# reonaledo/Multi-modality-Self-supervision

Hardware: AMD Instinct MI355X
Metric: image-text pairs/sec pretraining step, BERT-base seq512 (higher is better)
Workload: dtype f16

## Files before the change

include/medvill.h:

```cpp
#ifndef MEDVILL_H_
#define MEDVILL_H_

#include <stddef.h>
#include <stdint.h>

#ifdef __cplusplus
extern "C" {
#endif

#define MV_ABI_VERSION 6

enum { MV_F32 = 0, MV_BF16 = 1, MV_F16 = 2 };

enum {
  MV_OK = 0,
  MV_E_ARG = -1,
  MV_E_SHAPE = -2,
  MV_E_DTYPE = -3,
  MV_E_WORKSPACE = -4,
  MV_E_NO_RCCL = -5,
  MV_E_COMM_BASE = -1000
};

enum {
// ... 102 lines not shown

int mv_ce_fwd_bwd(const void* logits, int l_dtype, int ld, const int32_t* labels, int R, int V,
                  float* out, void* dlogits, int d_dtype, int ldd,
                  const float* grad_scale_dev, float grad_scale_host, const float* loss_scale_dev, void* stream);

int mv_gather_rows(int dtype, const void* src, int lds, const int32_t* rows, int R, int H,
                   void* dst, int ldd, void* stream);
int mv_scatter_rows(int dtype, const void* src, int lds, const int32_t* rows, int R, int H,
                    void* dst, int ldd, int accumulate, void* stream);

int mv_colsum(int dtype, const void* x, int ldx, int M, int N, float* out, int accumulate, const float* grad_unscale_dev,
              void* stream);
int mv_colsum_partials(const float* part, int P, int ld, int N, float* out, const float* grad_unscale_dev, void* stream);

int mv_add(int dtype, const void* a, const void* b, void* c, size_t n, void* stream);

int mv_dact(int dtype, int mode, const void* dy, const void* z, void* out, size_t n, void* stream);

int mv_cast2d(const void* src, int src_dtype, long long lds, void* dst, int dst_dtype, long long ldd,
              int rows, int cols, void* stream);

int mv_transpose(int dtype, const void* src, long long lds, void* dst, long long ldd, int rows, int cols, void* stream);

int mv_cast(const void* src, int src_dtype, void* dst, int dst_dtype, size_t n, void* stream);

int mv_nchw_to_nhwc(const float* src, void* dst, int dst_dtype, int B, int C, int H, int W, int Cp, void* stream);
int mv_im2col(int dtype, const void* src, int B, int H, int W, int C, int kh, int kw, int stride, int pad, void* dst, int ldk,
              void* stream);
int mv_conv2d(int dtype, const void* x, const void* w, void* y, int y_dtype, int B, int H, int W, int C, int O, int kh, int kw,
              int stride, int pad, const float* bias, int epi, const void* R, int r_dtype, void* stream);
int mv_col_stats(int dtype, const void* x, int ldx, int rows, int C, float* stats, void* stream);
int mv_bn_finalize(const float* stats, int C, long long rows, float eps, float momentum, float* mean, float* rstd,
                   float* running_mean, float* running_var, void* stream);
int mv_bn_act(int dtype, const void* x, int x_dtype, const float* mean, const float* rstd, const float* gamma, const float* beta,
              const void* residual, void* y, long long rows, int C, int relu, void* stream);
int mv_maxpool3x3s2(int dtype, const void* x, void* y, int B, int H, int W, int C, void* stream);

int mv_dropout_mask(float p_drop, unsigned long long drop_key, size_t n, uint8_t* keep, float* scale_out,
                    void* stream);

int mv_adamw_step(float* p, const float* g, float* m, float* v, void* shadow_bf16, void* shadow_f16, size_t n,
                  float lr, float beta1, float beta2, float eps, float weight_decay, int step,
                  int correct_bias, float grad_scale, const float* scaler_state, void* stream);

int mv_count_nonfinite(const float* x, size_t n, float* counter, void* stream);
int mv_scaler_update(float* state, int growth_interval, float growth, float backoff, float max_scale, float min_scale,
// ... 54 lines not shown
```

multi-modality-self-supervision_amd/_lib.py:

```python
from __future__ import annotations

import ctypes as C
import os

import torch

HERE = os.path.dirname(os.path.abspath(__file__))
LIB_PATH = os.environ.get("MV_LIB_PATH") or os.path.join(HERE, "libmedvill_hip.so")
DBG_LIB_PATH = os.environ.get("MV_DBG_LIB_PATH") or (LIB_PATH[:-3] + "_dbg.so")

MV_F32, MV_BF16, MV_F16 = 0, 1, 2
EPI_NONE, EPI_BIAS, EPI_BIAS_GELU, EPI_BIAS_RES, EPI_DGELU, EPI_RES, EPI_BIAS_TANH, EPI_BIAS_GELU_D, EPI_MUL, EPI_BIAS_RELU, EPI_BIAS_RES_RELU = range(11)
_ERR = {-1: "MV_E_ARG (null pointer / bad size)", -2: "MV_E_SHAPE (unsupported shape or alignment)",
        -3: "MV_E_DTYPE", -4: "MV_E_WORKSPACE (workspace too small)", -5: "MV_E_NO_RCCL (librccl could not be loaded)"}

vp, i32, i64, f32, sz, u64, f64 = C.c_void_p, C.c_int, C.c_longlong, C.c_float, C.c_size_t, C.c_ulonglong, C.c_double

PROTOTYPES = {
    "mv_abi_version": [],
    "mv_build_info": [],
    "mv_stream_create_cumask": [vp, i32, C.POINTER(C.c_void_p)],
    "mv_stream_destroy": [vp],
    "mv_comm_unique_id": [vp],
    "mv_comm_init": [C.POINTER(C.c_void_p), i32, i32, vp],
# ... 17 lines not shown
    "mv_pack_plan": [vp, i32, i32, vp, vp, vp, vp],
    "mv_tail_perm": [vp, i32, i32, vp, i32, vp, vp, vp, vp, vp],
    "mv_attn_fwd": [i32, vp, vp, vp, vp, vp, vp, i32, i32, i32, i32, f32, vp, vp, i32, vp, vp],
    "mv_attn_dropmask": [f32, u64, i32, i32, i32, vp, vp, vp],
    "mv_attn_bwd": [i32, vp, vp, vp, vp, vp, vp, vp, vp, i32, i32, i32, i32, f32, vp, vp, i32, vp, vp],
    "mv_attn_probs": [i32, vp, vp, vp, vp, vp, i32, i32, i32, i32, i32, f32, vp, i32, vp],
    "mv_layernorm_fwd": [i32, vp, i32, vp, vp, vp, vp, vp, vp, i32, i32, f32, vp],
    "mv_layernorm_bwd": [i32, vp, vp, i32, vp, vp, vp, vp, vp, vp, vp, i32, i32, vp, f32, u64, vp, vp],
    "mv_embed_fwd": [i32, vp, vp, vp, vp, vp, vp, vp, vp, vp, vp, vp, vp, vp, vp, vp, vp, i32, i32, i32, i32, i32, i32, f32, f32, f32,
                     u64, vp, i32, vp],
    "mv_embed_bwd": [i32, vp, vp, vp, vp, vp, vp, vp, vp, vp, vp, vp, vp, vp, vp, vp, vp, i32, i32, i32, i32, i32, i32, i32, f32, f32,
                     u64, vp, i32, vp, vp],
    "mv_dropout_mask": [f32, u64, sz, vp, C.POINTER(C.c_float), vp],
    "mv_ce_fwd_bwd": [vp, i32, i32, vp, i32, i32, vp, vp, i32, i32, vp, f32, vp, vp],
    "mv_gather_rows": [i32, vp, i32, vp, i32, i32, vp, i32, vp],
    "mv_scatter_rows": [i32, vp, i32, vp, i32, i32, vp, i32, i32, vp],
    "mv_colsum": [i32, vp, i32, i32, i32, vp, i32, vp, vp],
    "mv_colsum_partials": [vp, i32, i32, i32, vp, vp, vp],
    "mv_add": [i32, vp, vp, vp, sz, vp],
    "mv_dact": [i32, i32, vp, vp, vp, sz, vp],
    "mv_cast2d": [vp, i32, i64, vp, i32, i64, i32, i32, vp],
    "mv_cast": [vp, i32, vp, i32, sz, vp],
    "mv_transpose": [i32, vp, i64, vp, i64, i32, i32, vp],
    "mv_nchw_to_nhwc": [vp, vp, i32, i32, i32, i32, i32, i32, vp],
    "mv_im2col": [i32, vp, i32, i32, i32, i32, i32, i32, i32, i32, vp, i32, vp],
    "mv_conv2d": [i32, vp, vp, vp, i32, i32, i32, i32, i32, i32, i32, i32, i32, i32, vp, i32, vp, i32, vp],
    "mv_col_stats": [i32, vp, i32, i32, i32, vp, vp],
    "mv_bn_finalize": [vp, i32, i64, f32, f32, vp, vp, vp, vp, vp],
    "mv_bn_act": [i32, vp, i32, vp, vp, vp, vp, vp, vp, i64, i32, i32, vp],
    "mv_maxpool3x3s2": [i32, vp, vp, i32, i32, i32, i32, vp],
    "mv_adamw_step": [vp, vp, vp, vp, vp, vp, sz, f32, f32, f32, f32, f32, i32, i32, f32, vp, vp],
    "mv_count_nonfinite": [vp, sz, vp, vp],
    "mv_scaler_update": [vp, i32, f32, f32, f32, f32, vp],
    "mv_gemm_rows": [i32, i32, i32, i32, vp, i32, vp, i32, vp, i32, i32, vp, i32, vp, i32, i32, vp],
    "mv_attn_decode": [i32, vp, i32, vp, vp, i32, vp, i32, vp, vp, i32, vp, i32, i32, i32, i32, i32, vp, sz, vp],
    "mv_logprob_topk": [vp, i32, i32, i32, i32, i32, vp, vp, vp, vp],
    "mv_embed_rows": [i32, vp, vp, vp, vp, vp, vp, vp, vp, vp, i32, i32, i32, i32, i32, i32, f32, vp],
    "mv_bce_fwd_bwd": [vp, i32, vp, vp, i32, i32, vp, vp, i32, i32, vp, f32, vp, vp, vp, vp],
    "mv_rows_mul": [i32, vp, i32, vp, vp, i32, vp, i32, i32, vp, i32, vp],
    "mv_tensor_sqnorms": [vp, sz, vp, i32, vp, i32, vp, vp, vp],
    "mv_bce_multilabel": [vp, i32, vp, vp, i32, i32, vp, vp, i32, i32, vp, f32, vp, vp, vp, vp],
    "mv_bertadam_step": [vp, vp, vp, vp, vp, vp, sz, vp, i32, vp, i32, vp, f64, f64, f64, f32, f32, f32, i32, i32, f64, i32, vp, vp],
    "mv_lm_loss_fwd": [vp, i32, i32, i32, vp, vp, i32, f64, vp, vp, vp, vp],
    "mv_lm_loss_select": [vp, vp, vp, vp, i32, i32, i32, vp, vp, vp, vp],
    "mv_lm_loss_bwd": [vp, i32, i32, i32, vp, vp, vp, vp, i32, f64, vp, vp, vp, vp, vp, vp, i32, i32, vp],
    "mv_pair_draws": [u64, u64, i32, i32, vp, vp],
# ... 111 lines not shown
```

multi-modality-self-supervision_amd/csrc/mv_rowops.hip:

```cpp
#include "mv_common.h"

#define NC_DISPATCH(H_, CALL)                                  \
  do {                                                         \
    if ((H_) <= 256) { CALL(1); }                              \
    else if ((H_) <= 768) { CALL(3); }                         \
    else if ((H_) <= 1024) { CALL(4); }                        \
    else { CALL(8); }                                          \
  } while (0)
#define MV_MAX_H 2048

template <typename TX, typename TY, int NC>
__global__ __launch_bounds__(256) void ln_fwd_kernel(const TX* __restrict__ x, const float* __restrict__ g,
                                                     const float* __restrict__ bta, TY* __restrict__ y, float* __restrict__ mean,
                                                     float* __restrict__ rstd, int M, int H, float eps,
                                                     bf16_t* __restrict__ y_bf16) {
  const int lane = threadIdx.x & 63;
  const int row = blockIdx.x * 4 + (threadIdx.x >> 6);
  if (row >= M) return;
  const TX* xr = x + (size_t)row * H;
  f32x4 v[NC];
  float s = 0.f;
#pragma unroll
  for (int n = 0; n < NC; ++n) {
    const int c = lane * 4 + 256 * n;
// ... 191 lines not shown
  }
#pragma unroll
  for (int n = 0; n < NC; ++n) {
    const int c0 = 256 * n;
    if (c0 >= H) break;
#pragma unroll
    for (int e = 0; e < 4; ++e) { red[0][wl][lane * 4 + e] = ag[n][e]; red[1][wl][lane * 4 + e] = ab[n][e]; red[2][wl][lane * 4 + e] = ac[n][e]; }
    __syncthreads();
    const int t = threadIdx.x & 255;
    const int col = c0 + t;
    for (int which = threadIdx.x >> 8; which < 3; which += WPB / 4) {
      if (col < H && (which < 2 || colsum)) {
        const float gs = gscale ? *gscale : 1.0f;
        float a = 0.f;
#pragma unroll
        for (int w = 0; w < WPB; ++w) a += red[which][w][t];
        atomicAdd((which == 0 ? dgamma : which == 1 ? dbeta : colsum) + col, gs * a);
      }
    }
    __syncthreads();
  }
}

#define g_mv_ln_bwd_variant (mv_knob(MV_KNOB_ROWOPS_VARIANT))

extern "C" int mv_layernorm_fwd(int dtype, const void* x, int x_dtype, const float* gamma, const float* beta, void* y, void* y_bf16,
                                float* mean, float* rstd, int M, int H, float eps, void* stream_) {
  hipStream_t stream = (hipStream_t)stream_;
  if (!x || !gamma || !beta || !y || !mean || !rstd || M <= 0 || H <= 0) return MV_E_ARG;
  if ((H & 3) || H > MV_MAX_H) return MV_E_SHAPE;
  if (y_bf16 && dtype != MV_F16) return MV_E_DTYPE;
  dim3 grid((M + 3) / 4), block(256);
#define LNF(NC_) hipLaunchKernelGGL((ln_fwd_kernel<TX_, TY_, NC_>), grid, block, 0, stream, (const TX_*)x, gamma, beta, (TY_*)y, mean, rstd, M, H, eps, (bf16_t*)y_bf16)
  if (dtype == MV_F32 && x_dtype == MV_F32) { typedef float TX_; typedef float TY_; NC_DISPATCH(H, LNF); }
  else if (dtype == MV_BF16 && x_dtype == MV_F32) { typedef float TX_; typedef bf16_t TY_; NC_DISPATCH(H, LNF); }
  else if (dtype == MV_BF16 && x_dtype == MV_BF16) { typedef bf16_t TX_; typedef bf16_t TY_; NC_DISPATCH(H, LNF); }
  else if (dtype == MV_F16 && x_dtype == MV_F32) { typedef float TX_; typedef f16_t TY_; NC_DISPATCH(H, LNF); }
  else if (dtype == MV_F16 && x_dtype == MV_F16) { typedef f16_t TX_; typedef f16_t TY_; NC_DISPATCH(H, LNF); }
  else return MV_E_DTYPE;
#undef LNF
  MV_CHECK_LAUNCH();
  return MV_OK;
}

extern "C" int mv_layernorm_bwd(int dtype, const void* dy, const void* x, int x_dtype, const float* mean, const float* rstd,
                                const float* gamma, void* dx, float* dgamma, float* dbeta, float* colsum, int M, int H,
                                void* dx_drop, float p_drop, unsigned long long drop_key, const float* grad_unscale_dev, void* stream_) {
  hipStream_t stream = (hipStream_t)stream_;
  if (!dy || !x || !mean || !rstd || !gamma || !dx || !dgamma || !dbeta || M <= 0 || H <= 0) return MV_E_ARG;
  if ((H & 3) || H > MV_MAX_H) return MV_E_SHAPE;
  int var = g_mv_ln_bwd_variant & 0xff;
  if ((var == 0 || var == 3) && !(H <= 768 && x_dtype != MV_F32)) var = 2;
  const int wpb = var == 0 ? 8 : var == 3 ? 16 : 4;
  int blocks = (M + wpb - 1) / wpb;
  const int cap = (g_mv_ln_bwd_variant >> 8) > 0 ? (g_mv_ln_bwd_variant >> 8) : (var == 0 ? 512 : var == 3 ? 256 : 1024);
  if (blocks > cap) blocks = cap;
  dim3 grid(blocks), block(64 * wpb);
  const DropCfg drop = mv_make_drop(dx_drop ? p_drop : 0.f, drop_key);
  if (dx_drop && drop.thr == 0) dx_drop = nullptr;
#define LNB_ARGS (const TD_*)dy, (const TX_*)x, mean, rstd, gamma, (TD_*)dx, dgamma, dbeta, colsum, M, H, (TD_*)dx_drop, drop, grad_unscale_dev
#define LNB(NC_)                                                                                                                  \
  do {                                                                                                                            \
    constexpr bool wide_ok__ = (NC_) <= 3 && sizeof(TX_) == 2;                                                                    \
    if constexpr (wide_ok__) {                                                                                                    \
      if (var == 3) { hipLaunchKernelGGL((ln_bwd_pf_kernel<TX_, TD_, NC_, 16>), grid, block, 0, stream, LNB_ARGS); break; }       \
      if (var == 0) { hipLaunchKernelGGL((ln_bwd_pf_kernel<TX_, TD_, NC_, 8>), grid, block, 0, stream, LNB_ARGS); break; }        \
    }                                                                                                                             \
    if (var != 1) hipLaunchKernelGGL((ln_bwd_pf_kernel<TX_, TD_, NC_, 4>), grid, block, 0, stream, LNB_ARGS);                \
    else hipLaunchKernelGGL((ln_bwd_kernel<TX_, TD_, NC_>), grid, block, 0, stream, (const TD_*)dy, (const TX_*)x, mean, rstd, gamma, (TD_*)dx, dgamma, dbeta, colsum, M, H, (TD_*)dx_drop, drop, grad_unscale_dev); \
  } while (0)
  if (dtype == MV_F32 && x_dtype == MV_F32) { typedef float TX_; typedef float TD_; NC_DISPATCH(H, LNB); }
  else if (dtype == MV_BF16 && x_dtype == MV_F32) { typedef float TX_; typedef bf16_t TD_; NC_DISPATCH(H, LNB); }
  else if (dtype == MV_BF16 && x_dtype == MV_BF16) { typedef bf16_t TX_; typedef bf16_t TD_; NC_DISPATCH(H, LNB); }
  else if (dtype == MV_BF16 && x_dtype == MV_F16) { typedef f16_t TX_; typedef bf16_t TD_; NC_DISPATCH(H, LNB); }
  else if (dtype == MV_F16 && x_dtype == MV_F32) { typedef float TX_; typedef f16_t TD_; NC_DISPATCH(H, LNB); }
  else if (dtype == MV_F16 && x_dtype == MV_F16) { typedef f16_t TX_; typedef f16_t TD_; NC_DISPATCH(H, LNB); }
  else return MV_E_DTYPE;
#undef LNB
// ... 363 lines not shown
  if (drow) {
    const float gs = (gs_dev ? *gs_dev : gs_host) * (ls_dev ? *ls_dev : 1.0f);
    const float inv = gs / s;
#pragma unroll
    for (int n = 0; n < MAXV; ++n) {
      const int c = (tid + NT * n) * 4;
      if (c < ldd) {
        f32x4 o;
#pragma unroll
        for (int e = 0; e < 4; ++e) o[e] = (c + e < V) ? v[n][e] * inv - ((c + e) == label ? gs : 0.f) : 0.f;
        st4<TD>(drow + c, o);
      }
    }
  }
  __syncthreads();
  }
  if (tid == 0 && t_cnt > 0.f) {
    atomicAdd(out + 0, t_nll);
    atomicAdd(out + 1, t_cnt);
    if (t_ok > 0.f) atomicAdd(out + 2, t_ok);
  }
}

extern "C" int mv_ce_fwd_bwd(const void* logits, int l_dtype, int ld, const int32_t* labels, int R, int V, float* out, void* dlogits,
                             int d_dtype, int ldd, const float* grad_scale_dev, float grad_scale_host, const float* loss_scale_dev,
                             void* stream_) {
  hipStream_t stream = (hipStream_t)stream_;
  if (!logits || !labels || !out || R <= 0 || V <= 0 || ld < V) return MV_E_ARG;
  if (V > 256 * CE_MAXPER) return MV_E_SHAPE;
  if (dlogits && ldd < V) return MV_E_SHAPE;
  dim3 grid(R), block(256);
  const bool vec_ok = ((ld & 3) == 0) && (!dlogits || (ldd & 3) == 0) && ((((uintptr_t)logits) & 15) == 0) &&
                      (!dlogits || (((uintptr_t)dlogits) & 15) == 0) && V > 2048 && ldd <= 1024 * 32 && V <= 1024 * 32;
  if (vec_ok) {
    const dim3 vgrid(R < 512 ? R : 512), vblock(1024);
#define CEV_LAUNCH(TL, TD) hipLaunchKernelGGL((ce_vec_kernel<TL, TD, 8, 1024>), vgrid, vblock, 0, stream, (const TL*)logits, ld, labels, R, V, out, (TD*)dlogits, ldd, grad_scale_dev, grad_scale_host, loss_scale_dev)
    if (l_dtype == MV_F32 && d_dtype == MV_F32) CEV_LAUNCH(float, float);
    else if (l_dtype == MV_F32 && d_dtype == MV_F16) CEV_LAUNCH(float, f16_t);
    else if (l_dtype == MV_F32 && d_dtype == MV_BF16) CEV_LAUNCH(float, bf16_t);
    else if (l_dtype == MV_BF16 && d_dtype == MV_BF16) CEV_LAUNCH(bf16_t, bf16_t);
    else if (l_dtype == MV_BF16 && d_dtype == MV_F32) CEV_LAUNCH(bf16_t, float);
    else if (l_dtype == MV_F16 && d_dtype == MV_F16) CEV_LAUNCH(f16_t, f16_t);
    else if (l_dtype == MV_F16 && d_dtype == MV_F32) CEV_LAUNCH(f16_t, float);
    else return MV_E_DTYPE;
#undef CEV_LAUNCH
    MV_CHECK_LAUNCH();
    return MV_OK;
  }
#define CE_LAUNCH(TL, TD)                                                                                              \
  do {                                                                                                                 \
    if (V <= 256 * 8) hipLaunchKernelGGL((ce_kernel<TL, TD, 8>), grid, block, 0, stream, (const TL*)logits, ld, labels, R, V, out, (TD*)dlogits, ldd, grad_scale_dev, grad_scale_host, loss_scale_dev); \
    else hipLaunchKernelGGL((ce_kernel<TL, TD, CE_MAXPER>), grid, block, 0, stream, (const TL*)logits, ld, labels, R, V, out, (TD*)dlogits, ldd, grad_scale_dev, grad_scale_host, loss_scale_dev); \
  } while (0)
  if (l_dtype == MV_F32 && d_dtype == MV_F32) CE_LAUNCH(float, float);
  else if (l_dtype == MV_F32 && d_dtype == MV_F16) CE_LAUNCH(float, f16_t);
  else if (l_dtype == MV_F32 && d_dtype == MV_BF16) CE_LAUNCH(float, bf16_t);
  else if (l_dtype == MV_BF16 && d_dtype == MV_BF16) CE_LAUNCH(bf16_t, bf16_t);
  else if (l_dtype == MV_BF16 && d_dtype == MV_F32) CE_LAUNCH(bf16_t, float);
  else if (l_dtype == MV_F16 && d_dtype == MV_F16) CE_LAUNCH(f16_t, f16_t);
  else if (l_dtype == MV_F16 && d_dtype == MV_F32) CE_LAUNCH(f16_t, float);
  else return MV_E_DTYPE;
#undef CE_LAUNCH
  MV_CHECK_LAUNCH();
  return MV_OK;
}

template <typename T>
__global__ void gather_rows_kernel(const T* __restrict__ src, int lds_, const int32_t* __restrict__ rows, int R, int H,
// ... 230 lines not shown
  if (rows > 65535 * 16) return MV_E_SHAPE;
  int bx = (int)((ldd + 255) / 256);
  if (bx > 32) bx = 32;
  for (int r0 = 0; r0 < rows; r0 += 65535) {
    const int nr = rows - r0 < 65535 ? rows - r0 : 65535;
    dim3 grid(bx, nr), block(256);
    const char* sp = (const char*)src + (size_t)r0 * lds_ * mv_dtype_size(src_dtype);
    char* dp = (char*)dst + (size_t)r0 * ldd * mv_dtype_size(dst_dtype);
    if (src_dtype == MV_F32 && dst_dtype == MV_BF16) hipLaunchKernelGGL((cast2d_kernel<float, bf16_t>), grid, block, 0, stream, (const float*)sp, lds_, (bf16_t*)dp, ldd, nr, cols);
    else if (src_dtype == MV_BF16 && dst_dtype == MV_F32) hipLaunchKernelGGL((cast2d_kernel<bf16_t, float>), grid, block, 0, stream, (const bf16_t*)sp, lds_, (float*)dp, ldd, nr, cols);
    else if (src_dtype == MV_F32 && dst_dtype == MV_F32) hipLaunchKernelGGL((cast2d_kernel<float, float>), grid, block, 0, stream, (const float*)sp, lds_, (float*)dp, ldd, nr, cols);
    else if (src_dtype == MV_BF16 && dst_dtype == MV_BF16) hipLaunchKernelGGL((cast2d_kernel<bf16_t, bf16_t>), grid, block, 0, stream, (const bf16_t*)sp, lds_, (bf16_t*)dp, ldd, nr, cols);
    else if (src_dtype == MV_F32 && dst_dtype == MV_F16) hipLaunchKernelGGL((cast2d_kernel<float, f16_t>), grid, block, 0, stream, (const float*)sp, lds_, (f16_t*)dp, ldd, nr, cols);
    else if (src_dtype == MV_F16 && dst_dtype == MV_F32) hipLaunchKernelGGL((cast2d_kernel<f16_t, float>), grid, block, 0, stream, (const f16_t*)sp, lds_, (float*)dp, ldd, nr, cols);
    else if (src_dtype == MV_F16 && dst_dtype == MV_F16) hipLaunchKernelGGL((cast2d_kernel<f16_t, f16_t>), grid, block, 0, stream, (const f16_t*)sp, lds_, (f16_t*)dp, ldd, nr, cols);
    else return MV_E_DTYPE;
    MV_CHECK_LAUNCH();
  }
  return MV_OK;
}

template <typename T>
__global__ __launch_bounds__(256) void transpose_kernel(const T* __restrict__ src, long long lds_, T* __restrict__ dst, long long ldd,
                                                        int rows, int cols) {
  __shared__ T tile[64][65];
  const int tx = threadIdx.x & 63, ty = threadIdx.x >> 6;
  const int r0 = blockIdx.y * 64, c0 = blockIdx.x * 64;
#pragma unroll
  for (int i = 0; i < 16; ++i) {
    const int r = r0 + ty * 16 + i, c = c0 + tx;
    if (r < rows && c < cols) tile[ty * 16 + i][tx] = src[(size_t)r * lds_ + c];
  }
  __syncthreads();
#pragma unroll
  for (int i = 0; i < 16; ++i) {
    const int c = c0 + ty * 16 + i, r = r0 + tx;
    if (r < rows && c < cols) dst[(size_t)c * ldd + r] = tile[tx][ty * 16 + i];
  }
}
extern "C" int mv_transpose(int dtype, const void* src, long long lds_, void* dst, long long ldd, int rows, int cols, void* stream_) {
  hipStream_t stream = (hipStream_t)stream_;
  if (!src || !dst || rows <= 0 || cols <= 0 || lds_ < cols || ldd < rows) return MV_E_ARG;
  dim3 grid((cols + 63) / 64, (rows + 63) / 64), block(256);
  if (grid.y > 65535) return MV_E_SHAPE;
  if (dtype == MV_BF16 || dtype == MV_F16) hipLaunchKernelGGL(transpose_kernel<bf16_t>, grid, block, 0, stream, (const bf16_t*)src, lds_, (bf16_t*)dst, ldd, rows, cols);
  else if (dtype == MV_F32) hipLaunchKernelGGL(transpose_kernel<float>, grid, block, 0, stream, (const float*)src, lds_, (float*)dst, ldd, rows, cols);
  else return MV_E_DTYPE;
  MV_CHECK_LAUNCH();
  return MV_OK;
}

template <typename TS, typename TDs>
__global__ void cast_kernel(const TS* __restrict__ s, TDs* __restrict__ d, size_t n) {
  const size_t n4 = n / 4;
  for (size_t i = blockIdx.x * (size_t)blockDim.x + threadIdx.x; i < n4; i += (size_t)gridDim.x * blockDim.x)
    st4<TDs>(d + 4 * i, ld4<TS>(s + 4 * i));
  if (blockIdx.x == 0 && threadIdx.x < (n & 3)) stf<TDs>(d + n4 * 4 + threadIdx.x, ldf<TS>(s + n4 * 4 + threadIdx.x));
}
extern "C" int mv_cast(const void* src, int src_dtype, void* dst, int dst_dtype, size_t n, void* stream_) {
  hipStream_t stream = (hipStream_t)stream_;
  if (!src || !dst || n == 0) return MV_E_ARG;
  int blocks = (int)((n / 4 + 255) / 256);
  if (blocks > 2048) blocks = 2048;
  if (blocks < 1) blocks = 1;
  if (src_dtype == MV_F32 && dst_dtype == MV_BF16) hipLaunchKernelGGL((cast_kernel<float, bf16_t>), dim3(blocks), dim3(256), 0, stream, (const float*)src, (bf16_t*)dst, n);
  else if (src_dtype == MV_BF16 && dst_dtype == MV_F32) hipLaunchKernelGGL((cast_kernel<bf16_t, float>), dim3(blocks), dim3(256), 0, stream, (const bf16_t*)src, (float*)dst, n);
  else if (src_dtype == MV_F32 && dst_dtype == MV_F32) hipLaunchKernelGGL((cast_kernel<float, float>), dim3(blocks), dim3(256), 0, stream, (const float*)src, (float*)dst, n);
  else if (src_dtype == MV_BF16 && dst_dtype == MV_BF16) hipLaunchKernelGGL((cast_kernel<bf16_t, bf16_t>), dim3(blocks), dim3(256), 0, stream, (const bf16_t*)src, (bf16_t*)dst, n);
  else if (src_dtype == MV_F32 && dst_dtype == MV_F16) hipLaunchKernelGGL((cast_kernel<float, f16_t>), dim3(blocks), dim3(256), 0, stream, (const float*)src, (f16_t*)dst, n);
  else if (src_dtype == MV_F16 && dst_dtype == MV_F32) hipLaunchKernelGGL((cast_kernel<f16_t, float>), dim3(blocks), dim3(256), 0, stream, (const f16_t*)src, (float*)dst, n);
  else if (src_dtype == MV_F16 && dst_dtype == MV_BF16) hipLaunchKernelGGL((cast_kernel<f16_t, bf16_t>), dim3(blocks), dim3(256), 0, stream, (const f16_t*)src, (bf16_t*)dst, n);
  else if (src_dtype == MV_BF16 && dst_dtype == MV_F16) hipLaunchKernelGGL((cast_kernel<bf16_t, f16_t>), dim3(blocks), dim3(256), 0, stream, (const bf16_t*)src, (f16_t*)dst, n);
// ... 125 lines not shown
```

multi-modality-self-supervision_amd/engine.py:

```python
from __future__ import annotations

import math
import os
from collections import OrderedDict, namedtuple
from dataclasses import asdict, dataclass

import torch

from . import hip_ops as ops
from .data import MaskDesc
from ._lib import (EPI_BIAS, EPI_BIAS_GELU, EPI_BIAS_GELU_D, EPI_BIAS_RES, EPI_BIAS_TANH, EPI_MUL, EPI_NONE, EPI_RES, MV_BF16, MV_F16,
                   MV_F32)


@dataclass
class ModelConfig:
    vocab_size: int = 30522
    hidden: int = 768
    layers: int = 12
    heads: int = 12
    intermediate: int = 3072
    max_pos: int = 512
    type_vocab: int = 2
    img_hidden: int = 2048
# ... 128 lines not shown
        self.flat_p = torch.zeros(self.n_flat, dtype=torch.float32, device=self.device)
        self.flat_g = None
        self.flat_m = None
        self.flat_v = None
        self.shadow = torch.zeros(self.n_flat, dtype=torch.bfloat16, device=self.device) if MV_BF16 in (self.dt, self.fdt) else None
        self.shadow_f = torch.zeros(self.n_flat, dtype=torch.float16, device=self.device) if MV_F16 in (self.dt, self.fdt) else None
        self.scaler = None
        self.loss_scale_init = float(os.environ.get("MV_LOSS_SCALE", 2.0 ** 15))
        self.scale_growth_interval = 2000
        if self.dt == MV_F16:
            self.scaler = torch.zeros(8, dtype=torch.float32, device=self.device)
            self.reset_scaler()
        self.shadow_dirty = True
        self.S = {}
        self._ws = {}
        self._rows_now = self._rows_cap = 0
        self._gemm_ws = {}
        self._side = None
        self.training = False
        self.keep_acts = True
        self.attn_out = None
        self.ln_in_16 = os.environ.get("MV_LN_IN_16", "1") != "0"
        self.dz_nt = os.environ.get("MV_DZ_NT", "1") != "0"
        self._w2t, self._w2t_ev, self._w2t_stale = None, None, True
        self.fused_colsum = os.environ.get("MV_FUSED_COLSUM", "1") != "0"
        self.grouped_dw = os.environ.get("MV_GROUPED_DW", "1") != "0"
        self.grouped_dw_parts = max(0, int(os.environ.get("MV_GROUPED_DW_PARTS", "0")))
        self._dw_group = {}
        self.tail_queries = os.environ.get("MV_TAIL_QUERIES", "1") != "0"
        self._dE_ev = None
        self._opt_ev = None
        self.drop_seed = (torch.initial_seed() ^ 0x5DEECE66D) & 0xFFFFFFFFFFFFFFFF
        self.drop_counter = 0
        self._bind()

    def reset_scaler(self, scale=None):
        if self.scaler is None:
            return
        s0 = float(scale if scale is not None else self.loss_scale_init)
        self.scaler.copy_(torch.tensor([s0, 1.0 / s0, 0, 0, 0, 0, 0, 0], dtype=torch.float32))

    @property
    def loss_scale_dev(self):
        return None if self.scaler is None else self.scaler[0:1]

    @property
    def unscale_dev(self):
# ... 35 lines not shown
            self.wait_optimizer()
            torch.cuda.current_stream().synchronize()
        for k in ("flat_p", "flat_g", "flat_m", "flat_v", "shadow", "shadow_f", "scaler"):
            t = getattr(self, k)
            if t is not None:
                setattr(self, k, t.to(device))
        self.device = device
        self._ws.clear()
        self.shadow_dirty = True
        self._gemm_ws = {}
        self._dw_group = {}
        self._bind()
        return self

    def sync_shadow(self):
        self.wait_optimizer()
        if self.shadow is not None:
            ops.cast(self.flat_p, self.shadow, self.n_flat)
        if self.shadow_f is not None:
            ops.cast(self.flat_p, self.shadow_f, self.n_flat)
        self.shadow_dirty = False
        self._w2t_stale = True

    def _w2t_fill(self, l):
        cfg = self.cfg
        if self._w2t is None:
            self._w2t = [torch.empty((cfg.intermediate, cfg.hidden), dtype=self.adt, device=self.device) for _ in range(cfg.layers)]
        ops.transpose(self.w[f"enc.encoder.layer.{l}.output.dense.weight"], self._w2t[l], cfg.hidden, cfg.intermediate)

    def refresh_w2t(self, on_side=True):
        if not (self.dz_nt and self.is16):
            return
        main = torch.cuda.current_stream()
        side = self.side_stream() if on_side else main
        side.wait_stream(main)
        with torch.cuda.stream(side):
            for l in range(self.cfg.layers):
                self._w2t_fill(l)
            self._w2t_ev = self._done(side)
        self._w2t_stale = False

    def side_stream(self):
        if os.environ.get("MV_SINGLE_STREAM") == "1":
            return torch.cuda.current_stream()
        if self._side is None:
            self._side = _shared_stream(self.device, "side")
        return self._side

    def mask_stream(self):
        return _shared_stream(self.device, "mask")

# ... 635 lines not shown
            return
        phase("overflow_check")
        ops.count_nonfinite(self.flat_g, self.scaler[6:7])
        ops.scaler_update(self.scaler, growth_interval=self.scale_growth_interval)

    def adamw_step(self, step, lr=1e-5, betas=(0.9, 0.999), eps=1e-6, weight_decay=0.0, correct_bias=True, grad_scale=1.0,
                   overlap=False, use_scaler=False):
        self.ensure_opt()
        phase("optimizer")
        scaler_state = self.scaler if (use_scaler and self.scaler is not None) else None
        if not (overlap and self.device.type == "cuda") or self.side_stream() == torch.cuda.current_stream():
            self.wait_optimizer()
            ops.adamw_step(self.flat_p, self.flat_g, self.flat_m, self.flat_v, self.shadow, self.n_flat, lr, betas[0], betas[1], eps,
                           weight_decay, step, correct_bias, grad_scale, shadow_f16=self.shadow_f, scaler_state=scaler_state)
            self.shadow_dirty = False
            self.refresh_w2t()
            phase(None)
            return
        from .dist import bucket_ranges
        cfg = self.cfg
        ranges = bucket_ranges(self.layout, self.n_flat, cfg.layers)
        main, side = torch.cuda.current_stream(), self.side_stream()
        side.wait_stream(main)
        evs = {}
        word_end = self.layout["enc.txt_embeddings.position_embeddings.weight"][0]
        ranges["embeddings_rest"] = (word_end, ranges["embeddings"][1])
        ranges["embeddings"] = (ranges["embeddings"][0], word_end)
        with torch.cuda.stream(side):
            for name in ["embeddings_rest", "embeddings"] + [f"layer{l}" for l in range(cfg.layers)] + ["heads"]:
                s_, e_ = ranges[name]
                sl = slice(s_, e_)
                ops.adamw_step(self.flat_p[sl], self.flat_g[sl], self.flat_m[sl], self.flat_v[sl],
                               None if self.shadow is None else self.shadow[sl], e_ - s_, lr, betas[0], betas[1], eps,
                               weight_decay, step, correct_bias, grad_scale,
                               shadow_f16=None if self.shadow_f is None else self.shadow_f[sl], scaler_state=scaler_state)
                if self.dz_nt and self.is16 and name.startswith("layer"):
                    self._w2t_fill(int(name[5:]))
                evs[name] = self._done(side)
        self._opt_ev = evs
        self._w2t_ev, self._w2t_stale = evs["heads"], False
        self.shadow_dirty = False
        phase(None)

    def _wait_opt(self, name):
        if self._opt_ev:
            ev = self._opt_ev.pop(name, None)
            if ev is not None:
                torch.cuda.current_stream().wait_event(ev)

    def wait_optimizer(self):
        if self._opt_ev:
            for ev in self._opt_ev.values():
                torch.cuda.current_stream().wait_event(ev)
            self._opt_ev = None
```

multi-modality-self-supervision_amd/hip_ops.py:

```python
from __future__ import annotations

import ctypes

import torch

from . import _lib as L
from ._lib import (EPI_BIAS, EPI_BIAS_GELU, EPI_BIAS_GELU_D, EPI_BIAS_RELU, EPI_BIAS_RES, EPI_BIAS_RES_RELU, EPI_BIAS_TANH, EPI_DGELU,
                   EPI_MUL, EPI_NONE, EPI_RES, MV_BF16, MV_F16,
                   MV_F32)


def _lib():
    return L.load()


def gemm(a, b, c, *, ta=False, tb=False, M, N, K, lda=None, ldb=None, ldc=None, bias=None, epi=EPI_NONE, r=None, ldr=None,
         c2=None, ldc2=None, c3=None, ldc3=None, splitk=1, ws=None, accumulate=False, p_drop=0.0, drop_key=0, alpha=None, colsum_part=None):
    L.require_cuda(a, b, c, bias, r, c2, c3, ws, alpha, colsum_part)
    if colsum_part is not None and (colsum_part.dtype != torch.float32 or colsum_part.numel() < 2 * ((M + 255) // 256) * N):
        raise ValueError("colsum_part: f32 [2*ceil(M/256), N]")
    lda = lda if lda is not None else (M if ta else K)
    ldb = ldb if ldb is not None else (N if tb else K)
    ldc = ldc if ldc is not None else N
    ldr = ldr if ldr is not None else N
# ... 241 lines not shown
    L.check(rc, "mv_add")


def dact(mode, dy, z, out, n):
    rc = _lib().mv_dact(L.dt_of(dy), mode, L.ptr(dy), L.ptr(z), L.ptr(out), n, L.stream_ptr())
    L.check(rc, "mv_dact")


def cast(src, dst, n):
    rc = _lib().mv_cast(L.ptr(src), L.dt_of(src), L.ptr(dst), L.dt_of(dst), n, L.stream_ptr())
    L.check(rc, "mv_cast")


def transpose(src, dst, rows, cols, lds=None, ldd=None):
    L.require_cuda(src, dst)
    if src.dtype != dst.dtype:
        raise TypeError("transpose: dtypes differ")
    rc = _lib().mv_transpose(L.dt_of(src), L.ptr(src), lds if lds is not None else cols, L.ptr(dst), ldd if ldd is not None else rows,
                             rows, cols, L.stream_ptr())
    L.check(rc, "mv_transpose")
    return dst


def nchw_to_nhwc(src, dst, B, C, H, W, Cp):
    L.require_cuda(src, dst)
    if src.dtype != torch.float32:
        raise TypeError("nchw_to_nhwc: source pixels must be float32")
    rc = _lib().mv_nchw_to_nhwc(L.ptr(src), L.ptr(dst), L.dt_of(dst), B, C, H, W, Cp, L.stream_ptr())
    L.check(rc, "mv_nchw_to_nhwc")


def im2col(src, dst, B, H, W, C, kh, kw, stride, pad, ldk):
    L.require_cuda(src, dst)
    rc = _lib().mv_im2col(L.dt_of(src), L.ptr(src), B, H, W, C, kh, kw, stride, pad, L.ptr(dst), ldk, L.stream_ptr())
    L.check(rc, "mv_im2col")


def conv2d(x, w, y, B, H, W, C, O, kh, kw, stride, pad, bias=None, epi=EPI_NONE, r=None):
    L.require_cuda(x, w, y, bias, r)
    rc = _lib().mv_conv2d(L.dt_of(x), L.ptr(x), L.ptr(w), L.ptr(y), L.dt_of(y), B, H, W, C, O, kh, kw, stride, pad, L.ptr(bias), epi,
                          L.ptr(r), L.dt_of(r) if r is not None else 0, L.stream_ptr())
    L.check(rc, "mv_conv2d")


def col_stats(x, ldx, rows, C, stats):
    L.require_cuda(x, stats)
# ... 51 lines not shown
    import ctypes
    keep = torch.empty(n, dtype=torch.uint8, device=device)
    sc = ctypes.c_float(1.0)
    rc = _lib().mv_dropout_mask(float(p_drop), int(drop_key), n, L.ptr(keep), ctypes.byref(sc), L.stream_ptr())
    L.check(rc, "mv_dropout_mask")
    return keep, float(sc.value)


def set_impl(impl: int):
    L.set_knob("impl", 1 if impl else 0)


def get_impl() -> int:
    return L.get_knob("impl")


def set_attn_planes(planes: int):
    L.set_knob("attn_planes", planes if planes in (8, 12) else 16)


def attn_drop_prob(p_drop: float) -> float:
    n = L.get_knob("attn_planes")
    return round(p_drop * (1 << n)) / float(1 << n)


def set_rowops_variant(v: int = 0):
    L.set_knob("rowops_variant", v)


def set_gemm_rounds(on: int = 1):
    L.set_knob("gemm_rounds", 1 if on else 0)


def set_attn_fwd(variant: int = 0):
    L.set_knob("attn_fwd", variant)


def set_attn_order(order: int = 0):
    L.set_knob("attn_order", order)


class RcclComm:

    def __init__(self, rank: int, world: int, unique_id: bytes):
        import ctypes
        if len(unique_id) != 128:
# ... 425 lines not shown
```

Measured before the change: 2892.

## Add prefetching LayerNorm and CE kernels, vectorized and batched weight transpose

Adds a persistent LayerNorm forward kernel that prefetches the next row into registers while normalizing the current one. It also adds a similar prefetching cross-entropy kernel, a 16-bit transpose kernel that packs elements into 32-bit words for wider loads and stores, and a batched transpose that refreshes every layer's transposed FFN output weight in one launch after the optimizer. Together these aim to hide global load latency and cut kernel launch count. The batched W2T refill now waits until the last layer's optimizer update, which can reduce overlap with the next step. The old paths stay reachable through knob bits.

Result: no change. 2907 (median of 6 runs) (+0.5%).

```diff
diff --git a/include/medvill.h b/include/medvill.h
--- a/include/medvill.h
+++ b/include/medvill.h
@@ -148,6 +148,9 @@
 
 int mv_transpose(int dtype, const void* src, long long lds, void* dst, long long ldd, int rows, int cols, void* stream);
 
+int mv_transpose_batched(int dtype, const void* src, long long lds, long long src_stride, void* dst, long long ldd,
+                         long long dst_stride, int rows, int cols, int batch, void* stream);
+
 int mv_cast(const void* src, int src_dtype, void* dst, int dst_dtype, size_t n, void* stream);
 
 int mv_nchw_to_nhwc(const float* src, void* dst, int dst_dtype, int B, int C, int H, int W, int Cp, void* stream);
diff --git a/multi-modality-self-supervision_amd/_lib.py b/multi-modality-self-supervision_amd/_lib.py
--- a/multi-modality-self-supervision_amd/_lib.py
+++ b/multi-modality-self-supervision_amd/_lib.py
@@ -63,6 +63,7 @@
     "mv_cast2d": [vp, i32, i64, vp, i32, i64, i32, i32, vp],
     "mv_cast": [vp, i32, vp, i32, sz, vp],
     "mv_transpose": [i32, vp, i64, vp, i64, i32, i32, vp],
+    "mv_transpose_batched": [i32, vp, i64, i64, vp, i64, i64, i32, i32, i32, vp],
     "mv_nchw_to_nhwc": [vp, vp, i32, i32, i32, i32, i32, i32, vp],
     "mv_im2col": [i32, vp, i32, i32, i32, i32, i32, i32, i32, i32, vp, i32, vp],
     "mv_conv2d": [i32, vp, vp, vp, i32, i32, i32, i32, i32, i32, i32, i32, i32, i32, vp, i32, vp, i32, vp],
diff --git a/multi-modality-self-supervision_amd/csrc/mv_rowops.hip b/multi-modality-self-supervision_amd/csrc/mv_rowops.hip
--- a/multi-modality-self-supervision_amd/csrc/mv_rowops.hip
+++ b/multi-modality-self-supervision_amd/csrc/mv_rowops.hip
@@ -237,7 +237,84 @@
   }
 }
 
+template <typename TX, typename TY, int NC, int WPB>
+__global__ __launch_bounds__(64 * WPB) void ln_fwd_pf_kernel(const TX* __restrict__ x, const float* __restrict__ g,
+                                                             const float* __restrict__ bta, TY* __restrict__ y, float* __restrict__ mean,
+                                                             float* __restrict__ rstd, int M, int H, float eps,
+                                                             bf16_t* __restrict__ y_bf16) {
+  typedef typename raw4<TX>::type RX;
+  const int lane = threadIdx.x & 63;
+  f32x4 gg[NC], bb[NC];
+#pragma unroll
+  for (int n = 0; n < NC; ++n) {
+    const int c = lane * 4 + 256 * n;
+    gg[n] = (f32x4){0.f, 0.f, 0.f, 0.f}; bb[n] = gg[n];
+    if (c < H) { gg[n] = *(const f32x4*)(g + c); bb[n] = *(const f32x4*)(bta + c); }
+  }
+  const int stride = gridDim.x * WPB;
+  int row = blockIdx.x * WPB + (threadIdx.x >> 6);
+  RX rx[NC];
+  if (row < M) {
+#pragma unroll
+    for (int n = 0; n < NC; ++n) {
+      const int c = lane * 4 + 256 * n;
+      if (c < H) rx[n] = *(const RX*)(x + (size_t)row * H + c);
+    }
+  }
+  for (; row < M; row += stride) {
+    const int nrow = row + stride;
+    RX nx[NC];
+    if (nrow < M) {
+#pragma unroll
+      for (int n = 0; n < NC; ++n) {
+        const int c = lane * 4 + 256 * n;
+        if (c < H) nx[n] = *(const RX*)(x + (size_t)nrow * H + c);
+      }
+    }
+    f32x4 v[NC];
+    float s = 0.f;
+#pragma unroll
+    for (int n = 0; n < NC; ++n) {
+      const int c = lane * 4 + 256 * n;
+      v[n] = (f32x4){0.f, 0.f, 0.f, 0.f};
+      if (c < H) { v[n] = cvt_raw4<TX>(rx[n]); s += v[n][0] + v[n][1] + v[n][2] + v[n][3]; }
+    }
+    const float mu = wave_sum(s) / (float)H;
+    float q = 0.f;
+#pragma unroll
+    for (int n = 0; n < NC; ++n) {
+      if (lane * 4 + 256 * n < H) {
+#pragma unroll
+        for (int e = 0; e < 4; ++e) { const float d = v[n][e] - mu; q += d * d; }
+      }
+    }
+    const float var = wave_sum(q) / (float)H;
+    const float rs = 1.0f / sqrtf(var + eps);
+    TY* yr = y + (size_t)row * H;
+#pragma unroll
+    for (int n = 0; n < NC; ++n) {
+      const int c = lane * 4 + 256 * n;
+      if (c < H) {
+        f32x4 o;
+#pragma unroll
+        for (int e = 0; e < 4; ++e) o[e] = (v[n][e] - mu) * rs * gg[n][e] + bb[n][e];
+        st4<TY>(yr + c, o);
+        if (y_bf16) st4<bf16_t>(y_bf16 + (size_t)row * H + c, o);
+      }
+    }
+    if (lane == 0) { mean[row] = mu; rstd[row] = rs; }
+#pragma unroll
+    for (int n = 0; n < NC; ++n) rx[n] = nx[n];
+  }
+}
+
 #define g_mv_ln_bwd_variant (mv_knob(MV_KNOB_ROWOPS_VARIANT))
+#define MV_ROWOPS_CAP(v_) (((v_) >> 8) & 0xffff)
+#define MV_ROWOPS_OLD_LNF (1 << 24)
+#define MV_ROWOPS_OLD_TRANSPOSE (1 << 26)
+#define MV_ROWOPS_OLD_CE (1 << 27)
+#define MV_LNF_WPB 4
+#define MV_LNF_CAP 4096
 
 extern "C" int mv_layernorm_fwd(int dtype, const void* x, int x_dtype, const float* gamma, const float* beta, void* y, void* y_bf16,
                                 float* mean, float* rstd, int M, int H, float eps, void* stream_) {
@@ -245,8 +322,22 @@
   if (!x || !gamma || !beta || !y || !mean || !rstd || M <= 0 || H <= 0) return MV_E_ARG;
   if ((H & 3) || H > MV_MAX_H) return MV_E_SHAPE;
   if (y_bf16 && dtype != MV_F16) return MV_E_DTYPE;
+  const int knob = g_mv_ln_bwd_variant;
+  const int form = (knob >> 28) & 3;
+  const int wpb = form == 2 ? 8 : form == 1 ? 4 : MV_LNF_WPB;
+  int blocks = (M + wpb - 1) / wpb;
+  const int cap = (form && MV_ROWOPS_CAP(knob)) ? MV_ROWOPS_CAP(knob) : MV_LNF_CAP;
+  if (blocks > cap) blocks = cap;
+  const bool old_form = knob & MV_ROWOPS_OLD_LNF;
   dim3 grid((M + 3) / 4), block(256);
-#define LNF(NC_) hipLaunchKernelGGL((ln_fwd_kernel<TX_, TY_, NC_>), grid, block, 0, stream, (const TX_*)x, gamma, beta, (TY_*)y, mean, rstd, M, H, eps, (bf16_t*)y_bf16)
+  if (!old_form) { grid = dim3(blocks); block = dim3(64 * wpb); }
+#define LNF_ARGS (const TX_*)x, gamma, beta, (TY_*)y, mean, rstd, M, H, eps, (bf16_t*)y_bf16
+#define LNF(NC_)                                                                                                       \
+  do {                                                                                                                 \
+    if (old_form) hipLaunchKernelGGL((ln_fwd_kernel<TX_, TY_, NC_>), grid, block, 0, stream, LNF_ARGS);                \
+    else if (wpb == 8) hipLaunchKernelGGL((ln_fwd_pf_kernel<TX_, TY_, NC_, 8>), grid, block, 0, stream, LNF_ARGS);     \
+    else hipLaunchKernelGGL((ln_fwd_pf_kernel<TX_, TY_, NC_, 4>), grid, block, 0, stream, LNF_ARGS);                   \
+  } while (0)
   if (dtype == MV_F32 && x_dtype == MV_F32) { typedef float TX_; typedef float TY_; NC_DISPATCH(H, LNF); }
   else if (dtype == MV_BF16 && x_dtype == MV_F32) { typedef float TX_; typedef bf16_t TY_; NC_DISPATCH(H, LNF); }
   else if (dtype == MV_BF16 && x_dtype == MV_BF16) { typedef bf16_t TX_; typedef bf16_t TY_; NC_DISPATCH(H, LNF); }
@@ -254,6 +345,7 @@
   else if (dtype == MV_F16 && x_dtype == MV_F16) { typedef f16_t TX_; typedef f16_t TY_; NC_DISPATCH(H, LNF); }
   else return MV_E_DTYPE;
 #undef LNF
+#undef LNF_ARGS
   MV_CHECK_LAUNCH();
   return MV_OK;
 }
@@ -268,7 +360,7 @@
   if ((var == 0 || var == 3) && !(H <= 768 && x_dtype != MV_F32)) var = 2;
   const int wpb = var == 0 ? 8 : var == 3 ? 16 : 4;
   int blocks = (M + wpb - 1) / wpb;
-  const int cap = (g_mv_ln_bwd_variant >> 8) > 0 ? (g_mv_ln_bwd_variant >> 8) : (var == 0 ? 512 : var == 3 ? 256 : 1024);
+  const int cap = MV_ROWOPS_CAP(g_mv_ln_bwd_variant) > 0 ? MV_ROWOPS_CAP(g_mv_ln_bwd_variant) : (var == 0 ? 512 : var == 3 ? 256 : 1024);
   if (blocks > cap) blocks = cap;
   dim3 grid(blocks), block(64 * wpb);
   const DropCfg drop = mv_make_drop(dx_drop ? p_drop : 0.f, drop_key);
@@ -678,6 +770,118 @@
   }
 }
 
+template <typename TL, typename TD, int MAXV, int NT>
+__global__ __launch_bounds__(NT) void ce_vec_pf_kernel(const TL* __restrict__ logits, int ld, const int32_t* __restrict__ labels,
+                                                        int R, int V, float* __restrict__ out, TD* __restrict__ dlogits, int ldd,
+                                                        const float* __restrict__ gs_dev, float gs_host, const float* __restrict__ ls_dev) {
+  typedef typename raw4<TL>::type RL;
+  constexpr int NWV = NT / 64;
+  __shared__ float smax[NWV];
+  __shared__ int sarg[NWV];
+  __shared__ float ssum[NWV];
+  const int tid = threadIdx.x, lane = tid & 63, wl = tid >> 6;
+  float t_nll = 0.f, t_cnt = 0.f, t_ok = 0.f;
+  int row = blockIdx.x;
+  RL raw[MAXV];
+  int label = -1;
+  if (row < R) {
+    label = labels[row];
+#pragma unroll
+    for (int n = 0; n < MAXV; ++n) {
+      const int c = (tid + NT * n) * 4;
+      if (c < V) raw[n] = *(const RL*)(logits + (size_t)row * ld + c);
+    }
+  }
+  for (; row < R; row += gridDim.x) {
+    const int nrow = row + gridDim.x;
+    RL nraw[MAXV];
+    int nlabel = -1;
+    if (nrow < R) {
+      nlabel = labels[nrow];
+#pragma unroll
+      for (int n = 0; n < MAXV; ++n) {
+        const int c = (tid + NT * n) * 4;
+        if (c < V) nraw[n] = *(const RL*)(logits + (size_t)nrow * ld + c);
+      }
+    }
+    TD* drow = dlogits ? dlogits + (size_t)row * ldd : nullptr;
+    if (label < 0 || label >= V) {
+      if (drow) for (int c = tid * 4; c < ldd; c += NT * 4) st4<TD>(drow + c, (f32x4){0.f, 0.f, 0.f, 0.f});
+    } else {
+      const TL* lr = logits + (size_t)row * ld;
+      f32x4 v[MAXV];
+      float mx = -INFINITY;
+      int am = 0x7fffffff;
+#pragma unroll
+      for (int n = 0; n < MAXV; ++n) {
+        const int c = (tid + NT * n) * 4;
+        v[n] = (f32x4){-INFINITY, -INFINITY, -INFINITY, -INFINITY};
+        if (c < V) {
+          f32x4 x = cvt_raw4<TL>(raw[n]);
+#pragma unroll
+          for (int e = 0; e < 4; ++e) {
+            if (c + e >= V) x[e] = -INFINITY;
+            if (x[e] > mx) { mx = x[e]; am = c + e; }
+          }
+          v[n] = x;
+        }
+      }
+#pragma unroll
+      for (int o = 32; o > 0; o >>= 1) {
+        const float om = __shfl_xor(mx, o, 64);
+        const int oa = __shfl_xor(am, o, 64);
+        if (om > mx || (om == mx && oa < am)) { mx = om; am = oa; }
+      }
+      if (lane == 0) { smax[wl] = mx; sarg[wl] = am; }
+      __syncthreads();
+      mx = smax[0]; am = sarg[0];
+      for (int w = 1; w < NWV; ++w) if (smax[w] > mx || (smax[w] == mx && sarg[w] < am)) { mx = smax[w]; am = sarg[w]; }
+      float s = 0.f;
+      const float mxl = mx * 1.4426950408889634f;
+#pragma unroll
+      for (int n = 0; n < MAXV; ++n) {
+#pragma unroll
+        for (int e = 0; e < 4; ++e) { v[n][e] = fexp2(fmaf(v[n][e], 1.4426950408889634f, -mxl)); s += v[n][e]; }
+      }
+      s = wave_sum(s);
+      if (lane == 0) ssum[wl] = s;
+      __syncthreads();
+      s = 0.f;
+#pragma unroll
+      for (int w = 0; w < NWV; ++w) s += ssum[w];
+      if (tid == 0) {
+        const float xl = ldf<TL>(lr + label);
+        t_nll += (mx + logf(s)) - xl;
+        t_cnt += 1.0f;
+        if (am == label) t_ok += 1.0f;
+      }
+      if (drow) {
+        const float gs = (gs_dev ? *gs_dev : gs_host) * (ls_dev ? *ls_dev : 1.0f);
+        const float inv = gs / s;
+#pragma unroll
+        for (int n = 0; n < MAXV; ++n) {
+          const int c = (tid + NT * n) * 4;
+          if (c < ldd) {
+            f32x4 o;
+#pragma unroll
+            for (int e = 0; e < 4; ++e) o[e] = (c + e < V) ? v[n][e] * inv - ((c + e) == label ? gs : 0.f) : 0.f;
+            st4<TD>(drow + c, o);
+          }
+        }
+      }
+      __syncthreads();
+    }
+#pragma unroll
+    for (int n = 0; n < MAXV; ++n) raw[n] = nraw[n];
+    label = nlabel;
+  }
+  if (tid == 0 && t_cnt > 0.f) {
+    atomicAdd(out + 0, t_nll);
+    atomicAdd(out + 1, t_cnt);
+    if (t_ok > 0.f) atomicAdd(out + 2, t_ok);
+  }
+}
+
 extern "C" int mv_ce_fwd_bwd(const void* logits, int l_dtype, int ld, const int32_t* labels, int R, int V, float* out, void* dlogits,
                              int d_dtype, int ldd, const float* grad_scale_dev, float grad_scale_host, const float* loss_scale_dev,
                              void* stream_) {
@@ -690,7 +894,13 @@
                       (!dlogits || (((uintptr_t)dlogits) & 15) == 0) && V > 2048 && ldd <= 1024 * 32 && V <= 1024 * 32;
   if (vec_ok) {
     const dim3 vgrid(R < 512 ? R : 512), vblock(1024);
-#define CEV_LAUNCH(TL, TD) hipLaunchKernelGGL((ce_vec_kernel<TL, TD, 8, 1024>), vgrid, vblock, 0, stream, (const TL*)logits, ld, labels, R, V, out, (TD*)dlogits, ldd, grad_scale_dev, grad_scale_host, loss_scale_dev)
+    const bool old_form = g_mv_ln_bwd_variant & MV_ROWOPS_OLD_CE;
+#define CEV_ARGS(TL, TD) (const TL*)logits, ld, labels, R, V, out, (TD*)dlogits, ldd, grad_scale_dev, grad_scale_host, loss_scale_dev
+#define CEV_LAUNCH(TL, TD)                                                                                       \
+  do {                                                                                                           \
+    if (old_form) hipLaunchKernelGGL((ce_vec_kernel<TL, TD, 8, 1024>), vgrid, vblock, 0, stream, CEV_ARGS(TL, TD));      \
+    else hipLaunchKernelGGL((ce_vec_pf_kernel<TL, TD, 8, 1024>), vgrid, vblock, 0, stream, CEV_ARGS(TL, TD));            \
+  } while (0)
     if (l_dtype == MV_F32 && d_dtype == MV_F32) CEV_LAUNCH(float, float);
     else if (l_dtype == MV_F32 && d_dtype == MV_F16) CEV_LAUNCH(float, f16_t);
     else if (l_dtype == MV_F32 && d_dtype == MV_BF16) CEV_LAUNCH(float, bf16_t);
@@ -700,6 +910,7 @@
     else if (l_dtype == MV_F16 && d_dtype == MV_F32) CEV_LAUNCH(f16_t, float);
     else return MV_E_DTYPE;
 #undef CEV_LAUNCH
+#undef CEV_ARGS
     MV_CHECK_LAUNCH();
     return MV_OK;
   }
@@ -976,10 +1187,12 @@
 
 template <typename T>
 __global__ __launch_bounds__(256) void transpose_kernel(const T* __restrict__ src, long long lds_, T* __restrict__ dst, long long ldd,
-                                                        int rows, int cols) {
+                                                        int rows, int cols, long long src_stride, long long dst_stride) {
   __shared__ T tile[64][65];
   const int tx = threadIdx.x & 63, ty = threadIdx.x >> 6;
   const int r0 = blockIdx.y * 64, c0 = blockIdx.x * 64;
+  src += (size_t)blockIdx.z * src_stride;
+  dst += (size_t)blockIdx.z * dst_stride;
 #pragma unroll
   for (int i = 0; i < 16; ++i) {
     const int r = r0 + ty * 16 + i, c = c0 + tx;
@@ -992,16 +1205,62 @@
     if (r < rows && c < cols) dst[(size_t)c * ldd + r] = tile[tx][ty * 16 + i];
   }
 }
+__global__ __launch_bounds__(256) void transpose16_v4_kernel(const uint16_t* __restrict__ src, long long lds_, uint16_t* __restrict__ dst,
+                                                             long long ldd, int rows, int cols, long long src_stride,
+                                                             long long dst_stride) {
+  __shared__ uint32_t tile[64][33];
+  const int q = (threadIdx.x & 15) * 4, p = threadIdx.x >> 4;
+  const int r0 = blockIdx.y * 64, c0 = blockIdx.x * 64;
+  src += (size_t)blockIdx.z * src_stride;
+  dst += (size_t)blockIdx.z * dst_stride;
+#pragma unroll
+  for (int i = 0; i < 4; ++i) {
+    const int r = r0 + p + 16 * i, c = c0 + q;
+    if (r < rows && c < cols) {
+      const u32x2 v = *(const u32x2*)(src + (size_t)r * lds_ + c);
+      tile[p + 16 * i][q >> 1] = v[0];
+      tile[p + 16 * i][(q >> 1) + 1] = v[1];
+    }
+  }
+  __syncthreads();
+#pragma unroll
+  for (int i = 0; i < 4; ++i) {
+    const int c = c0 + p + 16 * i, r = r0 + q;
+    if (r < rows && c < cols) {
+      const int w = (p + 16 * i) >> 1, sh = 16 * (p & 1);
+      u32x2 v;
+      v[0] = ((tile[q][w] >> sh) & 0xffffu) | (((tile[q + 1][w] >> sh) & 0xffffu) << 16);
+      v[1] = ((tile[q + 2][w] >> sh) & 0xffffu) | (((tile[q + 3][w] >> sh) & 0xffffu) << 16);
+      *(u32x2*)(dst + (size_t)c * ldd + r) = v;
+    }
+  }
+}
+
+static int transpose_launch(int dtype, const void* src, long long lds_, void* dst, long long ldd, int rows, int cols, int batch,
+                            long long src_stride, long long dst_stride, hipStream_t stream) {
+  dim3 grid((cols + 63) / 64, (rows + 63) / 64, batch), block(256);
+  if (grid.y > 65535 || grid.z > 65535) return MV_E_SHAPE;
+  const bool v4 = !(g_mv_ln_bwd_variant & MV_ROWOPS_OLD_TRANSPOSE) && !((rows | cols | lds_ | ldd | src_stride | dst_stride) & 3) &&
+                  !((((uintptr_t)src) | ((uintptr_t)dst)) & 7);
+  if ((dtype == MV_BF16 || dtype == MV_F16) && v4)
+    hipLaunchKernelGGL(transpose16_v4_kernel, grid, block, 0, stream, (const uint16_t*)src, lds_, (uint16_t*)dst, ldd, rows, cols, src_stride, dst_stride);
+  else if (dtype == MV_BF16 || dtype == MV_F16)
+    hipLaunchKernelGGL(transpose_kernel<bf16_t>, grid, block, 0, stream, (const bf16_t*)src, lds_, (bf16_t*)dst, ldd, rows, cols, src_stride, dst_stride);
+  else if (dtype == MV_F32)
+    hipLaunchKernelGGL(transpose_kernel<float>, grid, block, 0, stream, (const float*)src, lds_, (float*)dst, ldd, rows, cols, src_stride, dst_stride);
+  else return MV_E_DTYPE;
+  MV_CHECK_LAUNCH();
+  return MV_OK;
+}
 extern "C" int mv_transpose(int dtype, const void* src, long long lds_, void* dst, long long ldd, int rows, int cols, void* stream_) {
-  hipStream_t stream = (hipStream_t)stream_;
   if (!src || !dst || rows <= 0 || cols <= 0 || lds_ < cols || ldd < rows) return MV_E_ARG;
-  dim3 grid((cols + 63) / 64, (rows + 63) / 64), block(256);
-  if (grid.y > 65535) return MV_E_SHAPE;
-  if (dtype == MV_BF16 || dtype == MV_F16) hipLaunchKernelGGL(transpose_kernel<bf16_t>, grid, block, 0, stream, (const bf16_t*)src, lds_, (bf16_t*)dst, ldd, rows, cols);
-  else if (dtype == MV_F32) hipLaunchKernelGGL(transpose_kernel<float>, grid, block, 0, stream, (const float*)src, lds_, (float*)dst, ldd, rows, cols);
-  else return MV_E_DTYPE;
-  MV_CHECK_LAUNCH();
-  return MV_OK;
+  return transpose_launch(dtype, src, lds_, dst, ldd, rows, cols, 1, 0, 0, (hipStream_t)stream_);
+}
+extern "C" int mv_transpose_batched(int dtype, const void* src, long long lds_, long long src_stride, void* dst, long long ldd,
+                                    long long dst_stride, int rows, int cols, int batch, void* stream_) {
+  if (!src || !dst || rows <= 0 || cols <= 0 || batch <= 0 || lds_ < cols || ldd < rows) return MV_E_ARG;
+  if (batch > 1 && (src_stride < (long long)(rows - 1) * lds_ + cols || dst_stride < (long long)(cols - 1) * ldd + rows)) return MV_E_ARG;
+  return transpose_launch(dtype, src, lds_, dst, ldd, rows, cols, batch, src_stride, dst_stride, (hipStream_t)stream_);
 }
 
 template <typename TS, typename TDs>
diff --git a/multi-modality-self-supervision_amd/engine.py b/multi-modality-self-supervision_amd/engine.py
--- a/multi-modality-self-supervision_amd/engine.py
+++ b/multi-modality-self-supervision_amd/engine.py
@@ -174,7 +174,8 @@
         self.attn_out = None
         self.ln_in_16 = os.environ.get("MV_LN_IN_16", "1") != "0"
         self.dz_nt = os.environ.get("MV_DZ_NT", "1") != "0"
-        self._w2t, self._w2t_ev, self._w2t_stale = None, None, True
+        self._w2t, self._w2t_all, self._w2t_ev, self._w2t_stale = None, None, None, True
+        self.batched_w2t = os.environ.get("MV_BATCHED_W2T", "1") != "0"
         self.fused_colsum = os.environ.get("MV_FUSED_COLSUM", "1") != "0"
         self.grouped_dw = os.environ.get("MV_GROUPED_DW", "1") != "0"
         self.grouped_dw_parts = max(0, int(os.environ.get("MV_GROUPED_DW_PARTS", "0")))
@@ -256,11 +257,25 @@
         self.shadow_dirty = False
         self._w2t_stale = True
 
+    def _w2t_alloc(self):
+        cfg = self.cfg
+        if self._w2t is None:
+            self._w2t_all = torch.empty((cfg.layers, cfg.intermediate, cfg.hidden), dtype=self.adt, device=self.device)
+            self._w2t = [self._w2t_all[l] for l in range(cfg.layers)]
+
     def _w2t_fill(self, l):
         cfg = self.cfg
-        if self._w2t is None:
-            self._w2t = [torch.empty((cfg.intermediate, cfg.hidden), dtype=self.adt, device=self.device) for _ in range(cfg.layers)]
+        self._w2t_alloc()
         ops.transpose(self.w[f"enc.encoder.layer.{l}.output.dense.weight"], self._w2t[l], cfg.hidden, cfg.intermediate)
+
+    def _w2t_fill_all(self):
+        cfg = self.cfg
+        self._w2t_alloc()
+        offs = [self.layout[f"enc.encoder.layer.{l}.output.dense.weight"][0] for l in range(cfg.layers)]
+        stride = offs[1] - offs[0] if cfg.layers > 1 else cfg.hidden * cfg.intermediate
+        assert all(offs[l] == offs[0] + l * stride for l in range(cfg.layers)), "layers are not equally spaced in the flat layout"
+        ops.transpose_batched(self.w["enc.encoder.layer.0.output.dense.weight"], self._w2t_all, cfg.hidden, cfg.intermediate, cfg.layers,
+                              stride, cfg.intermediate * cfg.hidden)
 
     def refresh_w2t(self, on_side=True):
         if not (self.dz_nt and self.is16):
@@ -942,7 +957,7 @@
         ranges = bucket_ranges(self.layout, self.n_flat, cfg.layers)
         main, side = torch.cuda.current_stream(), self.side_stream()
         side.wait_stream(main)
-        evs = {}
+        evs, w2t_ev = {}, None
         word_end = self.layout["enc.txt_embeddings.position_embeddings.weight"][0]
         ranges["embeddings_rest"] = (word_end, ranges["embeddings"][1])
         ranges["embeddings"] = (ranges["embeddings"][0], word_end)
@@ -954,11 +969,15 @@
                                None if self.shadow is None else self.shadow[sl], e_ - s_, lr, betas[0], betas[1], eps,
                                weight_decay, step, correct_bias, grad_scale,
                                shadow_f16=None if self.shadow_f is None else self.shadow_f[sl], scaler_state=scaler_state)
-                if self.dz_nt and self.is16 and name.startswith("layer"):
+                w2t = self.dz_nt and self.is16 and name.startswith("layer")
+                if w2t and not self.batched_w2t:
                     self._w2t_fill(int(name[5:]))
                 evs[name] = self._done(side)
+                if w2t and self.batched_w2t and name == f"layer{cfg.layers - 1}":
+                    self._w2t_fill_all()
+                    w2t_ev = self._done(side)
         self._opt_ev = evs
-        self._w2t_ev, self._w2t_stale = evs["heads"], False
+        self._w2t_ev, self._w2t_stale = (w2t_ev if w2t_ev is not None else evs["heads"]), False
         self.shadow_dirty = False
         phase(None)
 
diff --git a/multi-modality-self-supervision_amd/hip_ops.py b/multi-modality-self-supervision_amd/hip_ops.py
--- a/multi-modality-self-supervision_amd/hip_ops.py
+++ b/multi-modality-self-supervision_amd/hip_ops.py
@@ -287,6 +287,16 @@
     return dst
 
 
+def transpose_batched(src, dst, rows, cols, batch, src_stride, dst_stride, lds=None, ldd=None):
+    L.require_cuda(src, dst)
+    if src.dtype != dst.dtype:
+        raise TypeError("transpose_batched: dtypes differ")
+    rc = _lib().mv_transpose_batched(L.dt_of(src), L.ptr(src), lds if lds is not None else cols, int(src_stride), L.ptr(dst),
+                                     ldd if ldd is not None else rows, int(dst_stride), rows, cols, int(batch), L.stream_ptr())
+    L.check(rc, "mv_transpose_batched")
+    return dst
+
+
 def nchw_to_nhwc(src, dst, B, C, H, W, Cp):
     L.require_cuda(src, dst)
     if src.dtype != torch.float32:
@@ -384,6 +394,14 @@
 def attn_drop_prob(p_drop: float) -> float:
     n = L.get_knob("attn_planes")
     return round(p_drop * (1 << n)) / float(1 << n)
+
+
+ROWOPS_OLD_LN_FWD, ROWOPS_OLD_TRANSPOSE, ROWOPS_OLD_CE = 1 << 24, 1 << 26, 1 << 27
+ROWOPS_OLD_ALL = ROWOPS_OLD_LN_FWD | ROWOPS_OLD_TRANSPOSE | ROWOPS_OLD_CE
+
+
+def ln_fwd_form(waves_per_block: int, cap: int = 0) -> int:
+    return ({4: 1, 8: 2}[waves_per_block] << 28) | ((int(cap) & 0xffff) << 8)
 
 
 def set_rowops_variant(v: int = 0):
```
